# KDL-umass/CausalGPSLC.jl

Measured on AMD Instinct MI355X. Metric: posterior samples/sec (kernel+chol+predict) at N=4096; SATE rel-err vs CPU, higher is better.
Workload: dtype f64; 1 GPU; Synthetic N=4096 D=8 nU=2, unit A (Gram build + potrf + alpha + MeanITE + SATE mean/var), L=1 level(s), 1024 posterior samples per GPU per step; levels=1, mean_ite=True

## Files before the change

causalgpslc.jl_amd/csrc/k_tilegemm.hip:

```cpp
#include "gpslc_internal.h"
#include "diag_block.h"
#include "back_block.h"

typedef double d4 __attribute__((ext_vector_type(4)));
typedef double d2 __attribute__((ext_vector_type(2)));

#ifdef GPSLC_DIAG
#define GP_DBG_ON(g) ((g).dbg != nullptr)
#define GP_DIAG_SKIP(g) ((g).diag_skip)
#define GP_FENCE_MODE(a) ((a).fence_mode & 1)
#define GP_TASK_PRIO(a) (((a).fence_mode >> 4) & 3)
#define GP_TASK_WITHHOLD(a, b, is_diag, k) ((((a).fence_mode >> 6) & 1) && (b) == 0 && (is_diag) && (k) == 1)
#else
#define GP_DBG_ON(g) false
#define GP_DIAG_SKIP(g) 0
#define GP_FENCE_MODE(a) 0
#define GP_TASK_PRIO(a) 3
#define GP_TASK_WITHHOLD(a, b, is_diag, k) false
#endif

#define KLOOP_BARRIER asm volatile("s_waitcnt lgkmcnt(0)\n\ts_barrier" ::: "memory")
#define MFMA_PRIO_UP __builtin_amdgcn_s_setprio(1)
#define MFMA_PRIO_DOWN __builtin_amdgcn_s_setprio(0)

#define KS 16
#define LROW 144
#define OPER_LDS (KS * LROW)
#define GEMM_LDS_BYTES (2 * 2 * OPER_LDS * 8)
#ifndef SYRK_PF
#define SYRK_PF 2
#endif
#define FUSE_WD 8

__device__ __forceinline__ void tri_decode(int t, int& ii, int& jj) {
    int r = (int)((sqrt(8.0 * (double)t + 1.0) - 1.0) * 0.5);
    while ((long long)(r + 1) * (r + 2) / 2 <= t) ++r;
    while ((long long)r * (r + 1) / 2 > t) --r;
    ii = r;
    jj = t - r * (r + 1) / 2;
}

template <int NEG>
__device__ __forceinline__ d4 mfma_step(double a, double b, d4 c) {
    return __builtin_amdgcn_mfma_f64_16x16x4f64(a, b, c, 0, 0, NEG);
}

template <int ACC, int DIAG>
__global__ __launch_bounds__(256, 2) void tile_gemm_nt_kernel(GemmArgs g) {
    extern __shared__ __attribute__((aligned(16))) double smem[];
    const int tid = threadIdx.x;
    const int lane = tid & 63;
    const int wave = tid >> 6;
    const int wr = wave & 1, wc = wave >> 1;
    double* lA = smem;
    double* lB = smem + 2 * OPER_LDS;

    const long long W = (long long)g.ntiles * g.nbatch;
    const int G = gridDim.x;
    const int xcd = blockIdx.x & 7, local = blockIdx.x >> 3;
    const int gx = (G >> 3) + (xcd < (G & 7) ? 1 : 0);
    const long long wq = W >> 3, wrm = W & 7;
    const long long x0 = xcd * wq + (xcd < wrm ? xcd : wrm);
    const long long xc = wq + (xcd < wrm ? 1 : 0);

    const int crow = wr * 64 + (lane & 15);
    const int ccol = wc * 64 + (lane >> 4);
    const int frow_a = (lane >> 4) * LROW + wr * 64 + (lane & 15);
    const int frow_b = (lane >> 4) * LROW + wc * 64 + (lane & 15);
    int loff[4];
#pragma unroll
    for (int u = 0; u < 4; ++u) {
        const int q = tid + 256 * u;
        loff[u] = (q >> 6) * LROW + (q & 63) * 2;
    }
    const int nslab = (g.k1 - g.k0) * (GP_TS / KS);

    __shared__ int s_ticket;
    long long it = local;
    while (it < xc) {
        int ticket = 0;
        if (g.queue && tid == 0) ticket = atomicAdd(&g.queue[xcd], 1);
        do {
        const long long item = x0 + it;
        const int b = (int)(item / g.ntiles);
        const int t = (int)(item - (long long)b * g.ntiles);
        int ii, jj;
        if (g.order) { ii = g.order[2 * t]; jj = g.order[2 * t + 1]; }
        else if (g.shape == 0) tri_decode(t, ii, jj);
        else { ii = t / g.mj; jj = t - ii * g.mj; }
        const int ti = g.i0 + ii, tj = g.j0 + jj;
        if (g.sym >= 2 && ti == tj && !(g.short_rows > 0 && ti >= g.short_row0)) break;
        if (g.sym == 3 && g.short_rows > 0 && ti >= g.short_row0 && tj < g.short_row0) break;
        if (g.skip_gdiag && ti == tj && g.short_rows > 0 && ti >= g.short_row0) break;
        if (GP_DIAG_SKIP(g) == 3 && g.short_rows > 0 && ti >= g.short_row0) break;

        double* __restrict__ Ct = tref_tile(g.C, b, ti, tj);
        int mlive = 4;
        if (g.short_rows > 0 && ti >= g.short_row0) {
            const int mt = (g.short_rows + 15) >> 4;
            mlive = min(4, max(0, mt - 4 * wr));
        }
        const int pw = __builtin_amdgcn_readfirstlane(wave);
        int prow = 8;
        if (!ACC && g.short_rows > 0 && ti >= g.short_row0) prow = min(8, (g.short_rows + 15) >> 4);
        unsigned long long st0 = 0, st1 = 0, st2 = 0;
        if (GP_DBG_ON(g)) st0 = __builtin_amdgcn_s_memtime();

        d4 acc[4][4];
        if (ACC) {
            const double* __restrict__ Cl = Ct + (ccol * GP_TS + crow);
            if (g.nt_c) {
#pragma unroll
                for (int n = 0; n < 4; ++n)
#pragma unroll
                    for (int v = 0; v < 4; ++v)
#pragma unroll
                        for (int m = 0; m < 4; ++m)
                            acc[m][n][v] = __builtin_nontemporal_load(Cl + (16 * n + 4 * v) * GP_TS + 16 * m);
            } else {
#pragma unroll
                for (int n = 0; n < 4; ++n)
#pragma unroll
                    for (int v = 0; v < 4; ++v)
#pragma unroll
                        for (int m = 0; m < 4; ++m)
                            acc[m][n][v] = Cl[(16 * n + 4 * v) * GP_TS + 16 * m];
            }
        } else {
#pragma unroll
            for (int m = 0; m < 4; ++m)
#pragma unroll
                for (int n = 0; n < 4; ++n) acc[m][n] = (d4){0.0, 0.0, 0.0, 0.0};
        }

        if (nslab > 0) {
            d2 ra[4], rb[4];
            d2 ra2[4], rb2[4];
            auto gload = [&](int s, d2 (&xa)[4], d2 (&xb)[4]) {
                const int kk = g.k0 + (s >> 3);
                const int so = (s & 7) * (KS * GP_TS);
                const double* pa = tref_tile(g.A, b, ti, kk) + so;
                const double* pb = tref_tile(g.B, b, tj, kk) + so;
                const int ao = (!ACC && ((tid & 63) * 2) >= 16 * prow) ? (tid & ~63) * 2 : tid * 2;
#pragma unroll
                for (int u = 0; u < 4; ++u) {
                    xa[u] = *reinterpret_cast<const d2*>(pa + ao + 512 * u);
                    xb[u] = *reinterpret_cast<const d2*>(pb + (tid + 256 * u) * 2);
                }
            };
            auto lstore = [&](int buf, const d2 (&xa)[4], const d2 (&xb)[4]) {
#pragma unroll
                for (int u = 0; u < 4; ++u) {
                    *reinterpret_cast<d2*>(lA + buf * OPER_LDS + loff[u]) = xa[u];
                    *reinterpret_cast<d2*>(lB + buf * OPER_LDS + loff[u]) = xb[u];
                }
            };
            auto compute = [&](int buf, int s) {
                const double* pa = lA + buf * OPER_LDS + frow_a;
                const double* pb = lB + buf * OPER_LDS + frow_b;
                const int nlo = ACC ? 0 : min(4, max(0, (s & 7) - 4 * wc));
                constexpr bool PIPE = ACC && DIAG == 0;
                double afn[4], bfn[4];
                if (PIPE) {
#pragma unroll
                    for (int m = 0; m < 4; ++m) afn[m] = pa[16 * m];
#pragma unroll
                    for (int n = 0; n < 4; ++n) bfn[n] = pb[16 * n];
                }
#pragma unroll
                for (int ks = 0; ks < KS / 4; ++ks) {
                    double af[4], bf[4];
                    if (PIPE) {
#pragma unroll
                        for (int m = 0; m < 4; ++m) { af[m] = afn[m]; bf[m] = bfn[m]; }
                        if (ks + 1 < KS / 4) {
#pragma unroll
                            for (int m = 0; m < 4; ++m) afn[m] = pa[(ks + 1) * 4 * LROW + 16 * m];
#pragma unroll
                            for (int n = 0; n < 4; ++n) bfn[n] = pb[(ks + 1) * 4 * LROW + 16 * n];
                        }
                    } else {
#pragma unroll
                        for (int m = 0; m < 4; ++m) af[m] = pa[ks * 4 * LROW + 16 * m];
#pragma unroll
                        for (int n = 0; n < 4; ++n) bf[n] = pb[ks * 4 * LROW + 16 * n];
                    }
                    if (mlive == 4 && nlo == 0) {
#pragma unroll
                        for (int m = 0; m < 4; ++m)
#pragma unroll
                            for (int n = 0; n < 4; ++n)
                                acc[m][n] = mfma_step<ACC>(bf[n], af[m], acc[m][n]);
                    } else {
#pragma unroll
                        for (int m = 0; m < 4; ++m)
                            if (m < mlive) {
#pragma unroll
                                for (int n = 0; n < 4; ++n)
                                    if (n >= nlo) acc[m][n] = mfma_step<ACC>(bf[n], af[m], acc[m][n]);
                            }
                    }
                }
            };

            auto compute_p = [&](int buf, int s) {
                const int sl = s & 7;
                if (sl > 7 - pw) return;
                const bool use0 = sl <= pw;
                const double* pa = lA + buf * OPER_LDS + (lane >> 4) * LROW + (lane & 15);
                const double* pb = lB + buf * OPER_LDS + (lane >> 4) * LROW + (lane & 15);
#pragma unroll
                for (int ks = 0; ks < KS / 4; ++ks) {
                    const double b0 = pb[ks * 4 * LROW + 16 * pw];
                    const double b1 = pb[ks * 4 * LROW + 16 * (7 - pw)];
                    double af[8];
#pragma unroll
                    for (int m = 0; m < 8; ++m) af[m] = pa[ks * 4 * LROW + 16 * m];
#pragma unroll
                    for (int m = 0; m < 8; ++m)
                        if (m < prow) {
                            if (use0) acc[m >> 1][2 * (m & 1)] = mfma_step<0>(b0, af[m], acc[m >> 1][2 * (m & 1)]);
                            acc[m >> 1][2 * (m & 1) + 1] = mfma_step<0>(b1, af[m], acc[m >> 1][2 * (m & 1) + 1]);
                        }
                }
            };

            gload(0, ra, rb);
            lstore(0, ra, rb);
            gload(1, ra, rb);
            __syncthreads();
            if (GP_DBG_ON(g)) st1 = __builtin_amdgcn_s_memtime();
            if (DIAG == 0) {
                for (int s = 0; s < nslab; s += 2) {
                    if (s + 2 < nslab) gload(s + 2, ra2, rb2);
                    MFMA_PRIO_UP;
                    if (ACC) compute(0, s); else compute_p(0, s);
                    MFMA_PRIO_DOWN;
                    lstore(1, ra, rb);
                    KLOOP_BARRIER;
                    if (s + 3 < nslab) gload(s + 3, ra, rb);
                    MFMA_PRIO_UP;
                    if (ACC) compute(1, s + 1); else compute_p(1, s + 1);
                    MFMA_PRIO_DOWN;
                    if (s + 2 < nslab) lstore(0, ra2, rb2);
                    KLOOP_BARRIER;
                }
            } else {
                for (int s = 0; s < nslab; s += 2) {
                    compute(0, s);
                    if (DIAG == 1) lstore(1, ra, rb);
                    __syncthreads();
                    compute(1, s + 1);
                    if (DIAG == 1) lstore(0, ra, rb);
                    __syncthreads();
                }
            }
        }
        if (GP_DBG_ON(g)) st2 = __builtin_amdgcn_s_memtime();

        {
        if (!ACC) {
            double* __restrict__ Cp = Ct + ((lane >> 4) * GP_TS + (lane & 15));
#pragma unroll
            for (int m = 0; m < 8; ++m)
                if (m < prow) {
#pragma unroll
                    for (int v = 0; v < 4; ++v) {
                        Cp[(16 * pw + 4 * v) * GP_TS + 16 * m] = acc[m >> 1][2 * (m & 1)][v];
                        Cp[(16 * (7 - pw) + 4 * v) * GP_TS + 16 * m] = acc[m >> 1][2 * (m & 1) + 1][v];
                    }
                }
        } else {
        int soff = ccol * GP_TS + crow;
        asm volatile("" : "+v"(soff));
        double* __restrict__ Cs = Ct + soff;
        if (g.nt_c) {
#pragma unroll
            for (int n = 0; n < 4; ++n)
#pragma unroll
                for (int v = 0; v < 4; ++v)
#pragma unroll
                    for (int m = 0; m < 4; ++m)
                        __builtin_nontemporal_store(acc[m][n][v], Cs + (16 * n + 4 * v) * GP_TS + 16 * m);
        } else {
#pragma unroll
        for (int n = 0; n < 4; ++n)
#pragma unroll
            for (int v = 0; v < 4; ++v)
#pragma unroll
                for (int m = 0; m < 4; ++m)
                    Cs[(16 * n + 4 * v) * GP_TS + 16 * m] = acc[m][n][v];
        }
        }
        }
        if (GP_DBG_ON(g)) {
            asm volatile("s_waitcnt vmcnt(0)" ::: "memory");
            const unsigned long long st3 = __builtin_amdgcn_s_memtime();
            if (tid == 0) {
                unsigned long long* d = g.dbg + (size_t)item * 8;
                d[0] = st0; d[1] = st1; d[2] = st2; d[3] = st3;
                d[4] = __builtin_amdgcn_s_getreg((31 << 11) | 4);
                d[5] = __builtin_amdgcn_s_getreg((31 << 11) | 20);
                d[6] = __builtin_amdgcn_s_memrealtime();
                d[7] = blockIdx.x;
            }
        }
        } while (0);
        if (g.queue) {
            if (tid == 0) s_ticket = ticket;
            __syncthreads();
            it = (long long)gx + s_ticket;
            __syncthreads();
        } else {
            it += gx;
        }
    }
    if (g.queue && tid == 0) {
        __threadfence();
        if (atomicAdd(&g.queue[8 + xcd], 1) == gx - 1) {
            g.queue[xcd] = 0;
            g.queue[8 + xcd] = 0;
        }
    }
}

template <int WD, bool AUGEP = false, bool WT = false>
__device__ __forceinline__ void strip_item(const GemmArgs& g, const int b, const int ti, const int tj, const bool no_update,
                                           const int nslab, double* lA, double* lB, const int tid, const int lane,
                                           const int wave, const int li, const int lg, const int frow_a, const int frow_b,
                                           const int (&loff)[4], const long long item, const bool with_aug = false) {
    double* __restrict__ Ct = tref_tile(g.C, b, ti, tj);
    const bool live = !(g.short_rows > 0 && ti >= g.short_row0 && 32 * wave >= g.short_rows);
    unsigned long long st0 = 0, st1 = 0, st2 = 0;
    if (GP_DBG_ON(g)) st0 = __builtin_amdgcn_s_memtime();

    d4 acc[2][8];
    if (live) {
        const double* __restrict__ Cl = Ct + (lg * GP_TS + 32 * wave + li);
#pragma unroll
        for (int n = 0; n < 8; ++n)
#pragma unroll
            for (int v = 0; v < 4; ++v)
#pragma unroll
                for (int m = 0; m < 2; ++m)
                    acc[m][n][v] = __builtin_nontemporal_load(Cl + (16 * n + 4 * v) * GP_TS + 16 * m);
    }

    if (nslab > 0 && !no_update) {
        d2 ra[4], rb[4], ra2[4], rb2[4];
        auto gload = [&](int s, d2 (&xa)[4], d2 (&xb)[4]) {
            const int kk = g.k0 + (s >> 3);
            const int so = (s & 7) * (KS * GP_TS);
            const double* pa = tref_tile(g.A, b, ti, kk) + so;
            const double* pb = tref_tile(g.B, b, tj, kk) + so;
#pragma unroll
            for (int u = 0; u < 4; ++u) {
                xa[u] = __builtin_nontemporal_load(reinterpret_cast<const d2*>(pa + (tid + 256 * u) * 2));
                xb[u] = *reinterpret_cast<const d2*>(pb + (tid + 256 * u) * 2);
            }
        };
        auto lstore = [&](int buf, const d2 (&xa)[4], const d2 (&xb)[4]) {
#pragma unroll
            for (int u = 0; u < 4; ++u) {
                *reinterpret_cast<d2*>(lA + buf * OPER_LDS + loff[u]) = xa[u];
                *reinterpret_cast<d2*>(lB + buf * OPER_LDS + loff[u]) = xb[u];
            }
        };
        auto compute = [&](int buf) {
            if (!live) return;
            const double* pa = lA + buf * OPER_LDS + frow_a;
            const double* pb = lB + buf * OPER_LDS + frow_b;
#pragma unroll
            for (int ks = 0; ks < KS / 4; ++ks) {
                double af[2], bf[8];
#pragma unroll
                for (int m = 0; m < 2; ++m) af[m] = pa[ks * 4 * LROW + 16 * m];
#pragma unroll
                for (int n = 0; n < 8; ++n) bf[n] = pb[ks * 4 * LROW + 16 * n];
#pragma unroll
                for (int n = 0; n < 8; ++n)
#pragma unroll
                    for (int m = 0; m < 2; ++m) acc[m][n] = mfma_step<1>(bf[n], af[m], acc[m][n]);
            }
        };
        gload(0, ra, rb);
        lstore(0, ra, rb);
        gload(1, ra, rb);
        __syncthreads();
        if (GP_DBG_ON(g)) st1 = __builtin_amdgcn_s_memtime();
        for (int s = 0; s < nslab; s += 2) {
            if (s + 2 < nslab) gload(s + 2, ra2, rb2);
            compute(0);
            lstore(1, ra, rb);
            KLOOP_BARRIER;
            if (s + 3 < nslab) gload(s + 3, ra, rb);
            compute(1);
            if (s + 2 < nslab) lstore(0, ra2, rb2);
            KLOOP_BARRIER;
        }
    }
    if (GP_DBG_ON(g)) st2 = __builtin_amdgcn_s_memtime();

    if (live) {
        const double* __restrict__ Wl = tref_tile(g.F, b, 0, g.fk) + (lg * GP_TS + li);
        double* __restrict__ Co = Ct + (lg * GP_TS + 32 * wave + li);
        double wn[WD];
        int pc = 0, pn = 0, pv = 0;
#pragma unroll
        for (int q = 0; q < WD; ++q) {
            wn[q] = Wl[(16 * pn + 4 * pv) * GP_TS + 16 * pc];
            if (++pv == 4) { pv = 0; if (++pn > pc) { pn = 0; ++pc; } }
        }
        int q = 0;
#pragma unroll
        for (int nc = 0; nc < 8; ++nc) {
            d4 st[2];
            st[0] = (d4){0.0, 0.0, 0.0, 0.0};
            st[1] = (d4){0.0, 0.0, 0.0, 0.0};
#pragma unroll
            for (int n = 0; n < 8; ++n)
                if (n <= nc) {
#pragma unroll
                    for (int v = 0; v < 4; ++v) {
                        const double w = wn[q % WD];
                        if (pc < 8) {
                            wn[q % WD] = Wl[(16 * pn + 4 * pv) * GP_TS + 16 * pc];
                            if (++pv == 4) { pv = 0; if (++pn > pc) { pn = 0; ++pc; } }
                        }
                        ++q;
                        st[0] = mfma_step<0>(w, acc[0][n][v], st[0]);
                        st[1] = mfma_step<0>(w, acc[1][n][v], st[1]);
                    }
                }
#pragma unroll
            for (int v = 0; v < 4; ++v) {
                if (WT) {
                    out_store<true>(Co + (16 * nc + 4 * v) * GP_TS, st[0][v]);
                    out_store<true>(Co + (16 * nc + 4 * v) * GP_TS + 16, st[1][v]);
                } else {
                    __builtin_nontemporal_store(st[0][v], Co + (16 * nc + 4 * v) * GP_TS);
                    __builtin_nontemporal_store(st[1][v], Co + (16 * nc + 4 * v) * GP_TS + 16);
                }
            }
        }
    }
    if (AUGEP && with_aug) {
        const int mrows = (g.short_rows + 15) >> 4;
        double* __restrict__ Cg = tref_tile(g.C, b, g.short_row0, tj) + (lg * GP_TS + li);
        const double* __restrict__ Wl = tref_tile(g.F, b, 0, g.fk) + (lg * GP_TS + li);
        d4 ag[2][8];
#pragma unroll
        for (int n = 0; n < 8; ++n)
#pragma unroll
            for (int v = 0; v < 4; ++v)
#pragma unroll
                for (int m = 0; m < 2; ++m)
                    if (m < mrows) ag[m][n][v] = Cg[(16 * n + 4 * v) * GP_TS + 16 * m];
        auto colblock = [&](auto ncc) {
            constexpr int nc = decltype(ncc)::value;
            double wf[nc + 1][4];
#pragma unroll
            for (int n = 0; n <= nc; ++n)
#pragma unroll
                for (int v = 0; v < 4; ++v) wf[n][v] = Wl[(16 * n + 4 * v) * GP_TS + 16 * nc];
            d4 st[2];
            st[0] = (d4){0.0, 0.0, 0.0, 0.0};
            st[1] = (d4){0.0, 0.0, 0.0, 0.0};
#pragma unroll
            for (int n = 0; n <= nc; ++n)
#pragma unroll
                for (int v = 0; v < 4; ++v) {
                    st[0] = mfma_step<0>(wf[n][v], ag[0][n][v], st[0]);
                    if (mrows > 1) st[1] = mfma_step<0>(wf[n][v], ag[1][n][v], st[1]);
                }
#pragma unroll
            for (int v = 0; v < 4; ++v) {
                out_store<WT>(Cg + (16 * nc + 4 * v) * GP_TS, st[0][v]);
                if (mrows > 1) out_store<WT>(Cg + (16 * nc + 4 * v) * GP_TS + 16, st[1][v]);
            }
        };
        asm volatile("s_waitcnt vmcnt(0)" ::: "memory");
        __syncthreads();
        switch (wave) {
            case 0: colblock(std::integral_constant<int, 0>()); colblock(std::integral_constant<int, 7>()); break;
            case 1: colblock(std::integral_constant<int, 1>()); colblock(std::integral_constant<int, 6>()); break;
            case 2: colblock(std::integral_constant<int, 2>()); colblock(std::integral_constant<int, 5>()); break;
            default: colblock(std::integral_constant<int, 3>()); colblock(std::integral_constant<int, 4>()); break;
        }
    }
    if (GP_DBG_ON(g)) {
        asm volatile("s_waitcnt vmcnt(0)" ::: "memory");
        const unsigned long long st3 = __builtin_amdgcn_s_memtime();
        if (tid == 0) {
            unsigned long long* d = g.dbg + (size_t)item * 8;
            d[0] = st0; d[1] = st1; d[2] = st2; d[3] = st3;
            d[4] = __builtin_amdgcn_s_getreg((31 << 11) | 4);
            d[5] = __builtin_amdgcn_s_getreg((31 << 11) | 20);
            d[6] = __builtin_amdgcn_s_memrealtime();
            d[7] = blockIdx.x;
        }
    }
}

template <int WD>
__global__ __launch_bounds__(256, 2) void tile_fused_strip_kernel(GemmArgs g) {
    extern __shared__ __attribute__((aligned(16))) double smem[];
    const int tid = threadIdx.x;
    const int lane = tid & 63;
    const int wave = __builtin_amdgcn_readfirstlane(tid >> 6);
    const int li = lane & 15, lg = lane >> 4;
    double* lA = smem;
    double* lB = smem + 2 * OPER_LDS;

    const long long W = (long long)g.ntiles * g.nbatch;
    const int G = gridDim.x;
    const int xcd = blockIdx.x & 7, local = blockIdx.x >> 3;
    const int gx = (G >> 3) + (xcd < (G & 7) ? 1 : 0);
    const long long wq = W >> 3, wrm = W & 7;
    const long long x0 = xcd * wq + (xcd < wrm ? xcd : wrm);
    const long long xc = wq + (xcd < wrm ? 1 : 0);

    const int frow_a = lg * LROW + 32 * wave + li;
    const int frow_b = lg * LROW + li;
    int loff[4];
#pragma unroll
    for (int u = 0; u < 4; ++u) {
        const int q = tid + 256 * u;
        loff[u] = (q >> 6) * LROW + (q & 63) * 2;
    }
    const int nslab = (g.k1 - g.k0) * (GP_TS / KS);

    __shared__ int s_ticket;
    long long it = local;
    while (it < xc) {
        int ticket = 0;
        if (g.queue && tid == 0) ticket = atomicAdd(&g.queue[xcd], 1);
        do {
        const long long item = x0 + it;
        const int b = (int)(item / g.ntiles);
        const int t = (int)(item - (long long)b * g.ntiles);
        int ii, jj;
        if (g.shape == 0) tri_decode(t, ii, jj);
        else { ii = t / g.mj; jj = t - ii * g.mj; }
        const int ti = g.i0 + ii, tj = g.j0 + jj;
        if (g.sym >= 2 && ti == tj && !(g.short_rows > 0 && ti >= g.short_row0)) break;
        const bool no_update = g.sym == 3 && g.short_rows > 0 && ti >= g.short_row0 && tj < g.short_row0;
        strip_item<WD>(g, b, ti, tj, no_update, nslab, lA, lB, tid, lane, wave, li, lg, frow_a, frow_b, loff, item);
        } while (0);
        if (g.queue) {
            if (tid == 0) s_ticket = ticket;
            __syncthreads();
            it = (long long)gx + s_ticket;
            __syncthreads();
        } else {
            it += gx;
        }
    }
    if (g.queue && tid == 0) {
        __threadfence();
        if (atomicAdd(&g.queue[8 + xcd], 1) == gx - 1) {
            g.queue[xcd] = 0;
            g.queue[8 + xcd] = 0;
        }
    }
}

template <int W, int MT, bool WT = false>
__device__ __forceinline__ void syrk_chain_wave(const GemmArgs& g, const int b, const int td, const int kd1, double* smem,
                                                const int tid, const int lane) {
    double* lA = smem;
    double* lG = smem + 2 * OPER_LDS;
    int loff[4];
#pragma unroll
    for (int u = 0; u < 4; ++u) {
        const int q = tid + 256 * u;
        loff[u] = (q >> 6) * LROW + (q & 63) * 2;
    }
    const bool glive = MT > 0 && tid < 128 * MT;
    const int nslab = (kd1 - g.k0) * (GP_TS / KS);
    const int li = lane & 15, lg = lane >> 4;
    const int fbase = lg * LROW + li;
    double* __restrict__ Cd = tref_tile(g.C, b, td, td) + (lg * GP_TS + li);
    double* __restrict__ Cg = MT > 0 ? tref_tile(g.C, b, g.short_row0, td) + (lg * GP_TS + li) : nullptr;

    d4 a0c[W + 1], a1c[8 - W];
#pragma unroll
    for (int cb = 0; cb <= W; ++cb)
#pragma unroll
        for (int v = 0; v < 4; ++v) a0c[cb][v] = Cd[(16 * cb + 4 * v) * GP_TS + 16 * W];
#pragma unroll
    for (int cb = 0; cb < 8 - W; ++cb)
#pragma unroll
        for (int v = 0; v < 4; ++v) a1c[cb][v] = Cd[(16 * cb + 4 * v) * GP_TS + 16 * (7 - W)];
    d4 ag[MT > 0 ? MT : 1][2];
    if (MT > 0) {
#pragma unroll
        for (int m = 0; m < MT; ++m)
#pragma unroll
            for (int v = 0; v < 4; ++v) {
                ag[m][0][v] = Cg[(16 * W + 4 * v) * GP_TS + 16 * m];
                ag[m][1][v] = Cg[(16 * (7 - W) + 4 * v) * GP_TS + 16 * m];
            }
    }
    d2 rs[SYRK_PF][4], rgs[MT > 0 ? SYRK_PF : 1];
    const int gcol = tid / (8 * (MT > 0 ? MT : 1)), grp = tid % (8 * (MT > 0 ? MT : 1));
    auto gload = [&](int s, int set) {
        const int kk = g.k0 + (s >> 3);
        const double* pa = tref_tile(g.A, b, td, kk) + (s & 7) * (KS * GP_TS);
#pragma unroll
        for (int u = 0; u < 4; ++u) rs[set][u] = *reinterpret_cast<const d2*>(pa + (tid + 256 * u) * 2);
        if (MT > 0 && glive) {
            const double* pg = tref_tile(g.A, b, g.short_row0, kk) + (s & 7) * (KS * GP_TS);
            rgs[MT > 0 ? set : 0] = *reinterpret_cast<const d2*>(pg + gcol * GP_TS + 2 * grp);
        }
    };
    auto lstore = [&](int buf, int set) {
#pragma unroll
        for (int u = 0; u < 4; ++u) *reinterpret_cast<d2*>(lA + buf * OPER_LDS + loff[u]) = rs[set][u];
        if (MT > 0 && glive)
            *reinterpret_cast<d2*>(lG + buf * OPER_LDS + gcol * LROW + 2 * grp) = rgs[MT > 0 ? set : 0];
    };
    auto lds_barrier = [&]() { asm volatile("s_waitcnt lgkmcnt(0)\n\ts_barrier" ::: "memory"); };
    auto compute = [&](int buf) {
        const double* pa = lA + buf * OPER_LDS + fbase;
        const double* pg = lG + buf * OPER_LDS + fbase;
#pragma unroll
        for (int ks = 0; ks < KS / 4; ++ks) {
            double bf[8 - W];
#pragma unroll
            for (int cb = 0; cb < 8 - W; ++cb) bf[cb] = pa[ks * 4 * LROW + 16 * cb];
            const double r0 = pa[ks * 4 * LROW + 16 * W];
            const double r1 = pa[ks * 4 * LROW + 16 * (7 - W)];
#pragma unroll
            for (int cb = 0; cb <= W; ++cb) a0c[cb] = mfma_step<1>(bf[cb], r0, a0c[cb]);
#pragma unroll
            for (int cb = 0; cb < 8 - W; ++cb) a1c[cb] = mfma_step<1>(bf[cb], r1, a1c[cb]);
            if (MT > 0) {
#pragma unroll
                for (int m = 0; m < MT; ++m) {
                    const double gf = pg[ks * 4 * LROW + 16 * m];
                    ag[m][0] = mfma_step<1>(bf[W], gf, ag[m][0]);
                    ag[m][1] = mfma_step<1>(bf[7 - W], gf, ag[m][1]);
                }
            }
        }
    };
#pragma unroll
    for (int u = 0; u < SYRK_PF; ++u) gload(u, u);
    lstore(0, 0);
    lds_barrier();
    for (int s = 0; s < nslab; s += SYRK_PF) {
#pragma unroll
        for (int u = 0; u < SYRK_PF; ++u) {
            if (s + u + SYRK_PF < nslab) gload(s + u + SYRK_PF, u);
            compute(u & 1);
            if (s + u + 1 < nslab) lstore((u + 1) & 1, (u + 1) % SYRK_PF);
            lds_barrier();
        }
    }
    {
#pragma unroll
        for (int cb = 0; cb <= W; ++cb)
#pragma unroll
            for (int v = 0; v < 4; ++v) smem[(((W * (W + 1)) / 2 + cb) << 8) + (lg + 4 * v) * 16 + li] = a0c[cb][v];
#pragma unroll
        for (int cb = 0; cb < 8 - W; ++cb)
#pragma unroll
            for (int v = 0; v < 4; ++v) smem[((((7 - W) * (8 - W)) / 2 + cb) << 8) + (lg + 4 * v) * 16 + li] = a1c[cb][v];
    }
    if (MT > 0) {
#pragma unroll
        for (int m = 0; m < MT; ++m)
#pragma unroll
            for (int v = 0; v < 4; ++v) {
                out_store<WT>(Cg + (16 * W + 4 * v) * GP_TS + 16 * m, ag[m][0][v]);
                out_store<WT>(Cg + (16 * (7 - W) + 4 * v) * GP_TS + 16 * m, ag[m][1][v]);
            }
    }
}

template <int MT>
__global__ __launch_bounds__(256, 2) void diag_update_potrf_kernel(GemmArgs g) {
    extern __shared__ __attribute__((aligned(16))) double smem[];
    const int tid = threadIdx.x, lane = tid & 63;
    const int b = blockIdx.x;
    const int td = g.i0;
    switch (__builtin_amdgcn_readfirstlane(tid >> 6)) {
        case 0: syrk_chain_wave<0, MT>(g, b, td, g.k1, smem, tid, lane); break;
        case 1: syrk_chain_wave<1, MT>(g, b, td, g.k1, smem, tid, lane); break;
        case 2: syrk_chain_wave<2, MT>(g, b, td, g.k1, smem, tid, lane); break;
        default: syrk_chain_wave<3, MT>(g, b, td, g.k1, smem, tid, lane); break;
    }
    diag_potrf_inv_la_body(smem, tref_tile(g.C, b, td, td), tref_tile(g.F, b, 0, td), g.info + b, g.info_base + GP_TS * td,
                           tid, true);
}

template <int MT>
static void launch_diag_update_potrf_t(const GemmArgs& g, hipStream_t st) {
    static DeviceOnce once;
    constexpr int bytes = DIAG3_LDS_BYTES > GEMM_LDS_BYTES ? DIAG3_LDS_BYTES : GEMM_LDS_BYTES;
    lds_opt_in(once, (const void*)diag_update_potrf_kernel<MT>, bytes);
    hipLaunchKernelGGL(diag_update_potrf_kernel<MT>, dim3(g.nbatch), dim3(256), bytes, st, g);
}

void launch_diag_update_potrf(const GemmArgs& g, int carry_aug, hipStream_t st) {
    if (g.nbatch <= 0) return;
    const int mt = carry_aug ? (g.short_rows + 15) / 16 : 0;
    if (mt == 0) launch_diag_update_potrf_t<0>(g, st);
    else if (mt == 1) launch_diag_update_potrf_t<1>(g, st);
    else launch_diag_update_potrf_t<2>(g, st);
}

#define TASK_POLL_LIMIT (1 << 20)

__device__ __forceinline__ int task_progress_load(const int* p) {
    return __hip_atomic_load(p, __ATOMIC_RELAXED, __HIP_MEMORY_SCOPE_AGENT);
}
__device__ __forceinline__ void task_wait(const int* p, int need, int* tmo) {
    if (task_progress_load(p) >= need) return;
    for (int spins = 0;; ++spins) {
        __builtin_amdgcn_s_sleep(8);
        if (task_progress_load(p) >= need) return;
        if ((spins & 63) == 63 && task_progress_load(tmo) != 0) return;
        if (spins > TASK_POLL_LIMIT) {
            __hip_atomic_store(tmo, 1, __ATOMIC_RELAXED, __HIP_MEMORY_SCOPE_AGENT);
            return;
        }
    }
}

__device__ __forceinline__ unsigned task_fetch(const PotrfTaskArgs& a, int& q, int& visited) {
    while (visited < 8) {
        const int len = (int)a.list[8 + q];
        const int t = len > 0 ? atomicAdd(&a.sync[q], 1) : len;
        if (t < len) return a.list[TASK_LIST_HDR + a.list[q] + t];
        q = (q + 1) & 7;
        ++visited;
    }
    return TASK_NONE;
}

template <int MT, bool WT>
__global__ __launch_bounds__(256, 2) void potrf_tasks_kernel(PotrfTaskArgs a) {
    extern __shared__ __attribute__((aligned(16))) double smem[];
    __shared__ unsigned s_desc, s_next;
    __shared__ int s_q, s_visited;
    __shared__ unsigned long long s_ready;
    if (threadIdx.x == 0) {
        int q = (int)(__builtin_amdgcn_s_getreg((31 << 11) | 20) & 7);
        int visited = 0;
        s_next = task_fetch(a, q, visited);
        s_q = q; s_visited = visited;
    }
    for (;;) {
        int tid = threadIdx.x;
        asm volatile("" : "+v"(tid));
        unsigned long long stf = 0;
        if (GP_DBG_ON(a)) stf = __builtin_amdgcn_s_memtime();
        if (tid == 0) {
            int* const tmo = a.timeout;
            const unsigned d = s_next;
            if (d != TASK_NONE) {
                const int nt = a.nt;
                const int b = TASK_B(d), k = TASK_K(d), i = TASK_I(d), rows = TASK_ROWS(d);
                const int* prog = a.sync + TASK_SYNC_HDR + (long long)b * TASK_SYNC_STRIDE;
                if ((d >> 30) == 3) {
                    task_wait(prog, nt, tmo);
                    task_wait(prog + 1 + nt, nt, tmo);
                } else if ((d >> 30) & 1) {
                    if (k > 0) {
                        task_wait(prog + 1 + k, k, tmo);
                        if (MT > 0) task_wait(prog + 1 + nt, k, tmo);
                        if (rows > 1) task_wait(prog + 2 + k, k, tmo);
                    }
                } else {
                    task_wait(prog, k + 1, tmo);
                    if ((i < nt || MT == 0) && k > 0)
                        for (int r = 0; r < rows; ++r) task_wait(prog + 1 + i + r, k, tmo);
                }
                if (GP_DBG_ON(a)) s_ready = __builtin_amdgcn_s_memtime();
                __builtin_amdgcn_fence(__ATOMIC_ACQUIRE, "agent");
                asm volatile("s_waitcnt vmcnt(0)" ::: "memory");
            }
            s_desc = d;
        }
        __syncthreads();
        const unsigned d = s_desc;
        if (d == TASK_NONE) break;
        const int b = TASK_B(d), k = TASK_K(d), i = TASK_I(d), rows = TASK_ROWS(d);
        const bool is_back = (d >> 30) == 3;
        const bool is_diag = (d >> 30) == 1;
        const bool with_aug = (d >> 30) == 2;
        unsigned long long st0 = 0, st1 = 0;
        if (GP_DBG_ON(a)) st0 = __builtin_amdgcn_s_memtime();
        int tnext = 0, qn = 0, lenn = 0;
        if (tid == 0) {
            qn = s_q;
            lenn = s_visited < 8 ? (int)a.list[8 + qn] : 0;
            tnext = lenn > 0 ? atomicAdd(&a.sync[qn], 1) : 0;
        }
        const int lane = tid & 63;
        const int wave = __builtin_amdgcn_readfirstlane(tid >> 6);
        if (is_back) {
            back_task_body(a.g.C, a.g.F, b, a.nt, a.alpha + (long long)b * a.nt * GP_TS, smem, tid);
        } else if (is_diag) {
            if (GP_TASK_PRIO(a) == 3) __builtin_amdgcn_s_setprio(3);
            else if (GP_TASK_PRIO(a) == 1) __builtin_amdgcn_s_setprio(1);
            double* tile = tref_tile(a.g.C, b, k, k);
            double* invt = tref_tile(a.g.F, b, 0, k);
            if (k == 0) {
                diag_potrf_inv_la_body<WT>(smem, tile, invt, a.g.info + b, a.g.info_base, tid, false);
            } else {
                switch (wave) {
                    case 0: syrk_chain_wave<0, MT, WT>(a.g, b, k, k, smem, tid, lane); break;
                    case 1: syrk_chain_wave<1, MT, WT>(a.g, b, k, k, smem, tid, lane); break;
                    case 2: syrk_chain_wave<2, MT, WT>(a.g, b, k, k, smem, tid, lane); break;
                    default: syrk_chain_wave<3, MT, WT>(a.g, b, k, k, smem, tid, lane); break;
                }
                diag_potrf_inv_la_body<WT>(smem, tile, invt, a.g.info + b, a.g.info_base + GP_TS * k, tid, true);
            }
            __builtin_amdgcn_s_setprio(0);
        }
        const bool diag_then_strip = is_diag && rows > 1;
        if (diag_then_strip) {
            asm volatile("s_waitcnt vmcnt(0)" ::: "memory");
            __syncthreads();
        }
        if ((!is_diag && !is_back) || diag_then_strip) {
            const int li = lane & 15, lg = lane >> 4;
            int loff[4];
#pragma unroll
            for (int u = 0; u < 4; ++u) {
                const int q = tid + 256 * u;
                loff[u] = (q >> 6) * LROW + (q & 63) * 2;
            }
            GemmArgs gl = a.g;
            gl.k1 = k;
            gl.fk = k;
            if (diag_then_strip)
                strip_item<FUSE_WD, (MT > 0), WT>(gl, b, k + 1, k, false, 8 * k, smem, smem + 2 * OPER_LDS, tid, lane, wave, li, lg,
                                              lg * LROW + 32 * wave + li, lg * LROW + li, loff, 0, true);
            else
                for (int r = 0; r < rows; ++r)
                    strip_item<FUSE_WD, (MT > 0), WT>(gl, b, i + r, k, MT > 0 && i >= a.nt, 8 * k, smem, smem + 2 * OPER_LDS, tid,
                                                  lane, wave, li, lg, lg * LROW + 32 * wave + li, lg * LROW + li, loff, 0,
                                                  with_aug && r == 0);
        }
        asm volatile("s_waitcnt vmcnt(0)" ::: "memory");
        __syncthreads();
        if (GP_DBG_ON(a)) st1 = __builtin_amdgcn_s_memtime();
        if (tid == 0) {
            unsigned dn = TASK_NONE;
            const bool hit = tnext < lenn;
            if (hit) dn = a.list[TASK_LIST_HDR + a.list[qn] + tnext];
            int* prog = a.sync + TASK_SYNC_HDR + (long long)b * TASK_SYNC_STRIDE;
            if (!is_back && !GP_TASK_WITHHOLD(a, b, is_diag, k)) {
                if (GP_FENCE_MODE(a) == 0 && !WT) __builtin_amdgcn_fence(__ATOMIC_RELEASE, "agent");
                asm volatile("s_waitcnt vmcnt(0)" ::: "memory");
                if (is_diag) {
                    __hip_atomic_store(prog, k + 1, __ATOMIC_RELAXED, __HIP_MEMORY_SCOPE_AGENT);
                    if (diag_then_strip) {
                        __hip_atomic_store(prog + 2 + k, k + 1, __ATOMIC_RELAXED, __HIP_MEMORY_SCOPE_AGENT);
                        if (MT > 0) __hip_atomic_store(prog + 1 + a.nt, k + 1, __ATOMIC_RELAXED, __HIP_MEMORY_SCOPE_AGENT);
                    }
                } else
                    for (int r = 0; r < rows; ++r)
                        __hip_atomic_store(prog + 1 + i + r, k + 1, __ATOMIC_RELAXED, __HIP_MEMORY_SCOPE_AGENT);
                if (with_aug) __hip_atomic_store(prog + 1 + a.nt, k + 1, __ATOMIC_RELAXED, __HIP_MEMORY_SCOPE_AGENT);
            }
            if (!hit) {
                int q = qn, visited = s_visited;
                if (visited < 8) { q = (q + 1) & 7; ++visited; }
                dn = task_fetch(a, q, visited);
                s_q = q; s_visited = visited;
            }
            s_next = dn;
            if (GP_DBG_ON(a)) {
                unsigned long long* dd = a.dbg + 8 * (size_t)atomicAdd(a.sync + 9, 1);
                dd[0] = stf; dd[1] = st0; dd[2] = st1; dd[3] = __builtin_amdgcn_s_memtime(); dd[4] = d; dd[5] = blockIdx.x;
                dd[6] = s_ready; dd[7] = __builtin_amdgcn_s_getreg((31 << 11) | 20);
            }
        }
    }
}

template <int MT, bool WT>
static void launch_potrf_tasks_t(const PotrfTaskArgs& a, unsigned grid, hipStream_t st) {
    static DeviceOnce once;
    constexpr int bytes = DIAG3_LDS_BYTES > GEMM_LDS_BYTES ? DIAG3_LDS_BYTES : GEMM_LDS_BYTES;
    lds_opt_in(once, (const void*)potrf_tasks_kernel<MT, WT>, bytes);
    hipLaunchKernelGGL((potrf_tasks_kernel<MT, WT>), dim3(grid), dim3(256), bytes, st, a);
}

void launch_potrf_tasks(const PotrfTaskArgs& a, long long ntasks, int mt, hipStream_t st) {
    if (ntasks <= 0) return;
    int slots = 2 * device_cus();
#ifdef GPSLC_DIAG
    slots = diag_env("GPSLC_GEMM_SLOTS", slots);
#endif
    const unsigned grid = (unsigned)(ntasks < slots ? ntasks : slots);
#ifdef GPSLC_DIAG
    if (a.fence_mode & 2) {
        if (mt == 0) launch_potrf_tasks_t<0, false>(a, grid, st);
        else if (mt <= 1) launch_potrf_tasks_t<1, false>(a, grid, st);
        else launch_potrf_tasks_t<2, false>(a, grid, st);
        return;
    }
#endif
    if (mt == 0) launch_potrf_tasks_t<0, true>(a, grid, st);
    else if (mt <= 1) launch_potrf_tasks_t<1, true>(a, grid, st);
    else launch_potrf_tasks_t<2, true>(a, grid, st);
}

#define DG_LDS_BYTES(MT) ((2 * OPER_LDS + ((MT) > 0 ? 2 * OPER_LDS : 0)) * 8)

template <int W, int MT>
__device__ __forceinline__ void syrk_diag_wave(const GemmArgs& g, double* lA, int tid, int lane) {
    double* lG = lA + 2 * OPER_LDS;
    const long long Wk = (long long)g.mi * g.nbatch;
    const int G = gridDim.x;
    const int xcd = blockIdx.x & 7, local = blockIdx.x >> 3;
    const int gx = (G >> 3) + (xcd < (G & 7) ? 1 : 0);
    const long long wq = Wk >> 3, wrm = Wk & 7;
    const long long x0 = xcd * wq + (xcd < wrm ? xcd : wrm);
    const long long xc = wq + (xcd < wrm ? 1 : 0);
    int loff[4];
#pragma unroll
    for (int u = 0; u < 4; ++u) {
        const int q = tid + 256 * u;
        loff[u] = (q >> 6) * LROW + (q & 63) * 2;
    }
    const bool glive = MT > 0 && tid < 128 * MT;
    const int nslab = (g.k1 - g.k0) * (GP_TS / KS);
    const int fbase = (lane >> 4) * LROW + (lane & 15);

    for (long long it = local; it < xc; it += gx) {
        const long long item = x0 + it;
        const int b = (int)(item / g.mi);
        const int t = (int)(item - (long long)b * g.mi);
        const int ti = g.i0 + t;
        double* __restrict__ Cd = tref_tile(g.C, b, ti, ti) + ((lane >> 4) * GP_TS + (lane & 15));
        double* __restrict__ Cg = MT > 0 ? tref_tile(g.C, b, g.short_row0, ti) + ((lane >> 4) * GP_TS + (lane & 15)) : nullptr;

        d4 a0c[W + 1], a1c[8 - W];
#pragma unroll
        for (int cb = 0; cb <= W; ++cb)
#pragma unroll
            for (int v = 0; v < 4; ++v) a0c[cb][v] = Cd[(16 * cb + 4 * v) * GP_TS + 16 * W];
#pragma unroll
        for (int cb = 0; cb < 8 - W; ++cb)
#pragma unroll
            for (int v = 0; v < 4; ++v) a1c[cb][v] = Cd[(16 * cb + 4 * v) * GP_TS + 16 * (7 - W)];
        d4 ag[MT > 0 ? MT : 1][2];
        if (MT > 0) {
#pragma unroll
            for (int m = 0; m < MT; ++m)
#pragma unroll
                for (int v = 0; v < 4; ++v) {
                    ag[m][0][v] = Cg[(16 * W + 4 * v) * GP_TS + 16 * m];
                    ag[m][1][v] = Cg[(16 * (7 - W) + 4 * v) * GP_TS + 16 * m];
                }
        }

        d2 rs[SYRK_PF][4], rgs[MT > 0 ? SYRK_PF : 1];
        const int gcol = tid / (8 * (MT > 0 ? MT : 1)), grp = tid % (8 * (MT > 0 ? MT : 1));
        auto gload = [&](int s, int set) {
            const int kk = g.k0 + (s >> 3);
            const double* pa = tref_tile(g.A, b, ti, kk) + (s & 7) * (KS * GP_TS);
#pragma unroll
            for (int u = 0; u < 4; ++u) rs[set][u] = *reinterpret_cast<const d2*>(pa + (tid + 256 * u) * 2);
            if (MT > 0 && glive) {
                const double* pg = tref_tile(g.A, b, g.short_row0, kk) + (s & 7) * (KS * GP_TS);
                rgs[MT > 0 ? set : 0] = *reinterpret_cast<const d2*>(pg + gcol * GP_TS + 2 * grp);
            }
        };
        auto lstore = [&](int buf, int set) {
#pragma unroll
            for (int u = 0; u < 4; ++u) *reinterpret_cast<d2*>(lA + buf * OPER_LDS + loff[u]) = rs[set][u];
            if (MT > 0 && glive)
                *reinterpret_cast<d2*>(lG + buf * OPER_LDS + gcol * LROW + 2 * grp) = rgs[MT > 0 ? set : 0];
        };
        auto lds_barrier = [&]() { asm volatile("s_waitcnt lgkmcnt(0)\n\ts_barrier" ::: "memory"); };
        auto compute = [&](int buf) {
            const double* pa = lA + buf * OPER_LDS + fbase;
            const double* pg = lG + buf * OPER_LDS + fbase;
#pragma unroll
            for (int ks = 0; ks < KS / 4; ++ks) {
                double bf[8 - W];
#pragma unroll
                for (int cb = 0; cb < 8 - W; ++cb) bf[cb] = pa[ks * 4 * LROW + 16 * cb];
                const double r0 = pa[ks * 4 * LROW + 16 * W];
                const double r1 = pa[ks * 4 * LROW + 16 * (7 - W)];
#pragma unroll
                for (int cb = 0; cb <= W; ++cb) a0c[cb] = mfma_step<1>(bf[cb], r0, a0c[cb]);
#pragma unroll
                for (int cb = 0; cb < 8 - W; ++cb) a1c[cb] = mfma_step<1>(bf[cb], r1, a1c[cb]);
                if (MT > 0) {
#pragma unroll
                    for (int m = 0; m < MT; ++m) {
                        const double gf = pg[ks * 4 * LROW + 16 * m];
                        ag[m][0] = mfma_step<1>(bf[W], gf, ag[m][0]);
                        ag[m][1] = mfma_step<1>(bf[7 - W], gf, ag[m][1]);
                    }
                }
            }
        };
        if (nslab > 0) {
#pragma unroll
            for (int u = 0; u < SYRK_PF; ++u) gload(u, u);
            lstore(0, 0);
            lds_barrier();
            for (int s = 0; s < nslab; s += SYRK_PF) {
#pragma unroll
                for (int u = 0; u < SYRK_PF; ++u) {
                    if (s + u + SYRK_PF < nslab) gload(s + u + SYRK_PF, u);
                    compute(u & 1);
                    if (s + u + 1 < nslab) lstore((u + 1) & 1, (u + 1) % SYRK_PF);
                    lds_barrier();
                }
            }
        }
#pragma unroll
        for (int cb = 0; cb <= W; ++cb)
#pragma unroll
            for (int v = 0; v < 4; ++v) Cd[(16 * cb + 4 * v) * GP_TS + 16 * W] = a0c[cb][v];
#pragma unroll
        for (int cb = 0; cb < 8 - W; ++cb)
#pragma unroll
            for (int v = 0; v < 4; ++v) Cd[(16 * cb + 4 * v) * GP_TS + 16 * (7 - W)] = a1c[cb][v];
        if (MT > 0) {
#pragma unroll
            for (int m = 0; m < MT; ++m)
#pragma unroll
                for (int v = 0; v < 4; ++v) {
                    Cg[(16 * W + 4 * v) * GP_TS + 16 * m] = ag[m][0][v];
                    Cg[(16 * (7 - W) + 4 * v) * GP_TS + 16 * m] = ag[m][1][v];
                }
        }
    }
}

template <int MT>
__global__ __launch_bounds__(256, 2) void tile_syrk_diag_kernel(GemmArgs g) {
    extern __shared__ __attribute__((aligned(16))) double smem[];
    const int tid = threadIdx.x, lane = tid & 63;
    switch (__builtin_amdgcn_readfirstlane(tid >> 6)) {
        case 0: syrk_diag_wave<0, MT>(g, smem, tid, lane); break;
        case 1: syrk_diag_wave<1, MT>(g, smem, tid, lane); break;
        case 2: syrk_diag_wave<2, MT>(g, smem, tid, lane); break;
        default: syrk_diag_wave<3, MT>(g, smem, tid, lane); break;
    }
}

template <int MT>
static void launch_syrk_diag_t(const GemmArgs& g, unsigned grid, hipStream_t st) {
    static DeviceOnce once;
    lds_opt_in(once, (const void*)tile_syrk_diag_kernel<MT>, DG_LDS_BYTES(MT));
    hipLaunchKernelGGL(tile_syrk_diag_kernel<MT>, dim3(grid), dim3(256), DG_LDS_BYTES(MT), st, g);
}

void launch_syrk_diag(const GemmArgs& g, int carry_aug, hipStream_t st) {
    if (g.mi <= 0 || g.nbatch <= 0 || g.k1 <= g.k0) return;
    int slots = 2 * device_cus();
#ifdef GPSLC_DIAG
    slots = diag_env("GPSLC_GEMM_SLOTS", slots);
#endif
    const long long Wk = (long long)g.mi * g.nbatch;
    const unsigned grid = (unsigned)(Wk < slots ? Wk : slots);
    const int mt = carry_aug ? (g.short_rows + 15) / 16 : 0;
    if (mt == 0) launch_syrk_diag_t<0>(g, grid, st);
    else if (mt == 1) launch_syrk_diag_t<1>(g, grid, st);
    else launch_syrk_diag_t<2>(g, grid, st);
}

template <int ACC, int DIAG>
static void launch_one(const GemmArgs& g, unsigned grid, hipStream_t st) {
    static DeviceOnce once;
    lds_opt_in(once, (const void*)tile_gemm_nt_kernel<ACC, DIAG>, GEMM_LDS_BYTES);
    hipLaunchKernelGGL((tile_gemm_nt_kernel<ACC, DIAG>), dim3(grid), dim3(256), GEMM_LDS_BYTES, st, g);
}

void launch_tile_gemm(const GemmArgs& g, hipStream_t st) {
    if (g.ntiles <= 0 || g.nbatch <= 0) return;
    int slots = 2 * device_cus();
    const long long W = (long long)g.ntiles * g.nbatch;
#ifdef GPSLC_DIAG
    slots = diag_env("GPSLC_GEMM_SLOTS", slots);
    const int panel_slots = diag_env("GPSLC_PANEL_SLOTS", 0);
    if (!g.accumulate && panel_slots > 0) slots = panel_slots;
#endif
    const unsigned grid = (unsigned)(W < slots ? W : slots);
#ifdef GPSLC_DIAG
    if (g.diag_skip == 1) {
        if (g.accumulate) launch_one<1, 1>(g, grid, st); else launch_one<0, 1>(g, grid, st);
        return;
    }
    if (g.diag_skip == 2) {
        if (g.accumulate) launch_one<1, 2>(g, grid, st); else launch_one<0, 2>(g, grid, st);
        return;
    }
#endif
    if (g.fuse && g.accumulate) {
        static DeviceOnce once;
        lds_opt_in(once, (const void*)tile_fused_strip_kernel<FUSE_WD>, GEMM_LDS_BYTES);
        hipLaunchKernelGGL((tile_fused_strip_kernel<FUSE_WD>), dim3(grid), dim3(256), GEMM_LDS_BYTES, st, g);
    } else {
        if (g.accumulate) launch_one<1, 0>(g, grid, st); else launch_one<0, 0>(g, grid, st);
    }
}
```

Before: 2420 posterior samples/s.

## Load strip A operand directly to registers via buffer loads, halving LDS

The strip GEMM inner loop stops staging the A operand through LDS. Each wave now loads its own A fragments straight from global memory into registers with raw buffer loads, while B stays in double-buffered LDS. The lane mapping changes so each lane owns two adjacent columns, which lets C loads and stores use 128-bit accesses, and stores go through buffer stores. LDS per block is halved, which can raise occupancy and removes the A LDS writes and reads. The cost is more register pressure and a more complex prefetch schedule.

```diff
diff --git a/causalgpslc.jl_amd/csrc/k_tilegemm.hip b/causalgpslc.jl_amd/csrc/k_tilegemm.hip
--- a/causalgpslc.jl_amd/csrc/k_tilegemm.hip
+++ b/causalgpslc.jl_amd/csrc/k_tilegemm.hip
@@ -27,6 +27,7 @@
 #define LROW 144
 #define OPER_LDS (KS * LROW)
 #define GEMM_LDS_BYTES (2 * 2 * OPER_LDS * 8)
+#define STRIP_LDS_BYTES (2 * OPER_LDS * 8)
 #ifndef SYRK_PF
 #define SYRK_PF 2
 #endif
@@ -324,86 +325,129 @@
     }
 }
 
+typedef const __attribute__((address_space(1))) char* gcptr;
+__device__ __forceinline__ gcptr wave_uniform(const void* p) {
+    const unsigned long long x = (unsigned long long)p;
+    const unsigned lo = __builtin_amdgcn_readfirstlane((unsigned)x);
+    const unsigned hi = __builtin_amdgcn_readfirstlane((unsigned)(x >> 32));
+    return (gcptr)(((unsigned long long)hi << 32) | lo);
+}
+typedef unsigned u4 __attribute__((ext_vector_type(4)));
+template <bool WT>
+__device__ __forceinline__ void strip_store2(__amdgpu_buffer_rsrc_t rs, double* tile_lane, int lane_bytes, int col_doubles, d2 v) {
+    if (WT) __builtin_amdgcn_raw_buffer_store_b128(__builtin_bit_cast(u4, v), rs, lane_bytes + col_doubles * 8, 0,  16);
+    else __builtin_nontemporal_store(v, reinterpret_cast<d2*>(tile_lane + col_doubles));
+}
+
 template <int WD, bool AUGEP = false, bool WT = false>
 __device__ __forceinline__ void strip_item(const GemmArgs& g, const int b, const int ti, const int tj, const bool no_update,
-                                           const int nslab, double* lA, double* lB, const int tid, const int lane,
-                                           const int wave, const int li, const int lg, const int frow_a, const int frow_b,
+                                           const int nslab, double* lB, const int tid, const int lane,
+                                           const int wave, const int li, const int lg, const int frow_b,
                                            const int (&loff)[4], const long long item, const bool with_aug = false) {
     double* __restrict__ Ct = tref_tile(g.C, b, ti, tj);
     const bool live = !(g.short_rows > 0 && ti >= g.short_row0 && 32 * wave >= g.short_rows);
     unsigned long long st0 = 0, st1 = 0, st2 = 0;
     if (GP_DBG_ON(g)) st0 = __builtin_amdgcn_s_memtime();
+    const int lane_off = lg * GP_TS + 32 * wave + 2 * li;
 
     d4 acc[2][8];
     if (live) {
-        const double* __restrict__ Cl = Ct + (lg * GP_TS + 32 * wave + li);
+        const double* __restrict__ Cl = Ct + lane_off;
 #pragma unroll
         for (int n = 0; n < 8; ++n)
 #pragma unroll
-            for (int v = 0; v < 4; ++v)
-#pragma unroll
-                for (int m = 0; m < 2; ++m)
-                    acc[m][n][v] = __builtin_nontemporal_load(Cl + (16 * n + 4 * v) * GP_TS + 16 * m);
+            for (int v = 0; v < 4; ++v) {
+                const d2 c = __builtin_nontemporal_load(reinterpret_cast<const d2*>(Cl + (16 * n + 4 * v) * GP_TS));
+                acc[0][n][v] = c[0];
+                acc[1][n][v] = c[1];
+            }
     }
 
     if (nslab > 0 && !no_update) {
-        d2 ra[4], rb[4], ra2[4], rb2[4];
-        auto gload = [&](int s, d2 (&xa)[4], d2 (&xb)[4]) {
-            const int kk = g.k0 + (s >> 3);
-            const int so = (s & 7) * (KS * GP_TS);
-            const double* pa = tref_tile(g.A, b, ti, kk) + so;
-            const double* pb = tref_tile(g.B, b, tj, kk) + so;
-#pragma unroll
-            for (int u = 0; u < 4; ++u) {
-                xa[u] = __builtin_nontemporal_load(reinterpret_cast<const d2*>(pa + (tid + 256 * u) * 2));
-                xb[u] = *reinterpret_cast<const d2*>(pb + (tid + 256 * u) * 2);
-            }
+        constexpr int SLAB = KS * GP_TS * 8;
+        const int nsl = __builtin_amdgcn_readfirstlane(nslab);
+        const __amdgpu_buffer_rsrc_t rA = __builtin_amdgcn_make_buffer_rsrc(
+            (void*)(unsigned long long)wave_uniform(tref_tile(g.A, b, ti, g.k0)), 0, nsl * SLAB, 0x00020000);
+        const __amdgpu_buffer_rsrc_t rB = __builtin_amdgcn_make_buffer_rsrc(
+            (void*)(unsigned long long)wave_uniform(tref_tile(g.B, b, tj, g.k0)), 0, nsl * SLAB, 0x00020000);
+        int voa[4], vob[4];
+#pragma unroll
+        for (int u = 0; u < 4; ++u) {
+            voa[u] = (4 * u * GP_TS + lane_off) * 8;
+            vob[u] = (tid + 256 * u) * 16;
+        }
+        const std::true_type yes;
+        const std::false_type no;
+        auto kloop = [&](auto lv) {
+            constexpr bool LIVE = decltype(lv)::value;
+            d2 rb[4], rb2[4];
+            d2 a0[4], a1[4];
+            auto bload1 = [&](int so, int u) { return __builtin_bit_cast(d2, __builtin_amdgcn_raw_buffer_load_b128(rB, vob[u], so, 0)); };
+            auto bload = [&](int so, d2 (&xb)[4]) {
+#pragma unroll
+                for (int u = 0; u < 4; ++u) xb[u] = bload1(so, u);
+            };
+            auto aload = [&](int so, int ks) {
+                return __builtin_bit_cast(d2, __builtin_amdgcn_raw_buffer_load_b128(rA, voa[ks], so,  2));
+            };
+            auto lstore = [&](int buf, const d2 (&xb)[4]) {
+#pragma unroll
+                for (int u = 0; u < 4; ++u) *reinterpret_cast<d2*>(lB + buf * OPER_LDS + loff[u]) = xb[u];
+            };
+            auto slab = [&](auto pf, int buf, d2 (&aa)[4], int so, d2 (&lb)[4], auto ws, int wbuf,
+                            const d2 (&wb)[4]) {
+                constexpr bool PF = decltype(pf)::value;
+                constexpr bool WS = decltype(ws)::value;
+                const double* pb = lB + buf * OPER_LDS + frow_b;
+#pragma unroll
+                for (int ks = 0; ks < KS / 4; ++ks) {
+                    if (LIVE) {
+                        double bf[8];
+#pragma unroll
+                        for (int n = 0; n < 8; ++n) bf[n] = pb[ks * 4 * LROW + 16 * n];
+                        const d2 a = aa[ks];
+#pragma unroll
+                        for (int n = 0; n < 8; ++n)
+#pragma unroll
+                            for (int m = 0; m < 2; ++m) acc[m][n] = mfma_step<1>(bf[n], a[m], acc[m][n]);
+                        if (PF) aa[ks] = aload(so, ks);
+                    }
+                    if (PF) lb[ks] = bload1(so, ks);
+                    if (WS) *reinterpret_cast<d2*>(lB + wbuf * OPER_LDS + loff[ks]) = wb[ks];
+                }
+            };
+            bload(0, rb);
+            if (LIVE) {
+#pragma unroll
+                for (int ks = 0; ks < 4; ++ks) a0[ks] = aload(0, ks);
+#pragma unroll
+                for (int ks = 0; ks < 4; ++ks) a1[ks] = aload(SLAB, ks);
+            }
+            lstore(0, rb);
+            bload(SLAB, rb);
+            KLOOP_BARRIER;
+            if (GP_DBG_ON(g)) st1 = __builtin_amdgcn_s_memtime();
+            int so = 2 * SLAB;
+            for (int s = 0; s + 2 < nsl; s += 2) {
+                slab(yes, 0, a0, so, rb2, yes, 1, rb);
+                KLOOP_BARRIER;
+                slab(yes, 1, a1, so + SLAB, rb, yes, 0, rb2);
+                KLOOP_BARRIER;
+                so += 2 * SLAB;
+            }
+            slab(no, 0, a0, 0, rb2, yes, 1, rb);
+            KLOOP_BARRIER;
+            slab(no, 1, a1, 0, rb, no, 0, rb2);
+            KLOOP_BARRIER;
         };
-        auto lstore = [&](int buf, const d2 (&xa)[4], const d2 (&xb)[4]) {
-#pragma unroll
-            for (int u = 0; u < 4; ++u) {
-                *reinterpret_cast<d2*>(lA + buf * OPER_LDS + loff[u]) = xa[u];
-                *reinterpret_cast<d2*>(lB + buf * OPER_LDS + loff[u]) = xb[u];
-            }
-        };
-        auto compute = [&](int buf) {
-            if (!live) return;
-            const double* pa = lA + buf * OPER_LDS + frow_a;
-            const double* pb = lB + buf * OPER_LDS + frow_b;
-#pragma unroll
-            for (int ks = 0; ks < KS / 4; ++ks) {
-                double af[2], bf[8];
-#pragma unroll
-                for (int m = 0; m < 2; ++m) af[m] = pa[ks * 4 * LROW + 16 * m];
-#pragma unroll
-                for (int n = 0; n < 8; ++n) bf[n] = pb[ks * 4 * LROW + 16 * n];
-#pragma unroll
-                for (int n = 0; n < 8; ++n)
-#pragma unroll
-                    for (int m = 0; m < 2; ++m) acc[m][n] = mfma_step<1>(bf[n], af[m], acc[m][n]);
-            }
-        };
-        gload(0, ra, rb);
-        lstore(0, ra, rb);
-        gload(1, ra, rb);
-        __syncthreads();
-        if (GP_DBG_ON(g)) st1 = __builtin_amdgcn_s_memtime();
-        for (int s = 0; s < nslab; s += 2) {
-            if (s + 2 < nslab) gload(s + 2, ra2, rb2);
-            compute(0);
-            lstore(1, ra, rb);
-            KLOOP_BARRIER;
-            if (s + 3 < nslab) gload(s + 3, ra, rb);
-            compute(1);
-            if (s + 2 < nslab) lstore(0, ra2, rb2);
-            KLOOP_BARRIER;
-        }
+        if (live) kloop(yes); else kloop(no);
     }
     if (GP_DBG_ON(g)) st2 = __builtin_amdgcn_s_memtime();
 
     if (live) {
         const double* __restrict__ Wl = tref_tile(g.F, b, 0, g.fk) + (lg * GP_TS + li);
-        double* __restrict__ Co = Ct + (lg * GP_TS + 32 * wave + li);
+        double* __restrict__ Co = Ct + lane_off;
+        const __amdgpu_buffer_rsrc_t crs = __builtin_amdgcn_make_buffer_rsrc((void*)(unsigned long long)wave_uniform(Ct), 0, GP_TSQ * 8, 0x00020000);
         double wn[WD];
         int pc = 0, pn = 0, pv = 0;
 #pragma unroll
@@ -433,15 +477,8 @@
                     }
                 }
 #pragma unroll
-            for (int v = 0; v < 4; ++v) {
-                if (WT) {
-                    out_store<true>(Co + (16 * nc + 4 * v) * GP_TS, st[0][v]);
-                    out_store<true>(Co + (16 * nc + 4 * v) * GP_TS + 16, st[1][v]);
-                } else {
-                    __builtin_nontemporal_store(st[0][v], Co + (16 * nc + 4 * v) * GP_TS);
-                    __builtin_nontemporal_store(st[1][v], Co + (16 * nc + 4 * v) * GP_TS + 16);
-                }
-            }
+            for (int v = 0; v < 4; ++v)
+                strip_store2<WT>(crs, Co, lane_off * 8, (16 * nc + 4 * v) * GP_TS, (d2){st[0][v], st[1][v]});
         }
     }
     if (AUGEP && with_aug) {
@@ -509,8 +546,7 @@
     const int lane = tid & 63;
     const int wave = __builtin_amdgcn_readfirstlane(tid >> 6);
     const int li = lane & 15, lg = lane >> 4;
-    double* lA = smem;
-    double* lB = smem + 2 * OPER_LDS;
+    double* lB = smem;
 
     const long long W = (long long)g.ntiles * g.nbatch;
     const int G = gridDim.x;
@@ -520,7 +556,6 @@
     const long long x0 = xcd * wq + (xcd < wrm ? xcd : wrm);
     const long long xc = wq + (xcd < wrm ? 1 : 0);
 
-    const int frow_a = lg * LROW + 32 * wave + li;
     const int frow_b = lg * LROW + li;
     int loff[4];
 #pragma unroll
@@ -545,7 +580,7 @@
         const int ti = g.i0 + ii, tj = g.j0 + jj;
         if (g.sym >= 2 && ti == tj && !(g.short_rows > 0 && ti >= g.short_row0)) break;
         const bool no_update = g.sym == 3 && g.short_rows > 0 && ti >= g.short_row0 && tj < g.short_row0;
-        strip_item<WD>(g, b, ti, tj, no_update, nslab, lA, lB, tid, lane, wave, li, lg, frow_a, frow_b, loff, item);
+        strip_item<WD>(g, b, ti, tj, no_update, nslab, lB, tid, lane, wave, li, lg, frow_b, loff, item);
         } while (0);
         if (g.queue) {
             if (tid == 0) s_ticket = ticket;
@@ -838,13 +873,12 @@
             gl.k1 = k;
             gl.fk = k;
             if (diag_then_strip)
-                strip_item<FUSE_WD, (MT > 0), WT>(gl, b, k + 1, k, false, 8 * k, smem, smem + 2 * OPER_LDS, tid, lane, wave, li, lg,
-                                              lg * LROW + 32 * wave + li, lg * LROW + li, loff, 0, true);
+                strip_item<FUSE_WD, (MT > 0), WT>(gl, b, k + 1, k, false, 8 * k, smem, tid, lane, wave, li, lg, lg * LROW + li, loff, 0,
+                                              true);
             else
                 for (int r = 0; r < rows; ++r)
-                    strip_item<FUSE_WD, (MT > 0), WT>(gl, b, i + r, k, MT > 0 && i >= a.nt, 8 * k, smem, smem + 2 * OPER_LDS, tid,
-                                                  lane, wave, li, lg, lg * LROW + 32 * wave + li, lg * LROW + li, loff, 0,
-                                                  with_aug && r == 0);
+                    strip_item<FUSE_WD, (MT > 0), WT>(gl, b, i + r, k, MT > 0 && i >= a.nt, 8 * k, smem, tid, lane, wave, li, lg,
+                                                  lg * LROW + li, loff, 0, with_aug && r == 0);
         }
         asm volatile("s_waitcnt vmcnt(0)" ::: "memory");
         __syncthreads();
@@ -1102,8 +1136,8 @@
 #endif
     if (g.fuse && g.accumulate) {
         static DeviceOnce once;
-        lds_opt_in(once, (const void*)tile_fused_strip_kernel<FUSE_WD>, GEMM_LDS_BYTES);
-        hipLaunchKernelGGL((tile_fused_strip_kernel<FUSE_WD>), dim3(grid), dim3(256), GEMM_LDS_BYTES, st, g);
+        lds_opt_in(once, (const void*)tile_fused_strip_kernel<FUSE_WD>, STRIP_LDS_BYTES);
+        hipLaunchKernelGGL((tile_fused_strip_kernel<FUSE_WD>), dim3(grid), dim3(256), STRIP_LDS_BYTES, st, g);
     } else {
         if (g.accumulate) launch_one<1, 0>(g, grid, st); else launch_one<0, 0>(g, grid, st);
     }
```

Result: faster. 2499 posterior samples/s, median of 6 (+3.3%).
